# taekkii/deblurgs

Measured on AMD Instinct MI355X. Metric: subframe-renders/sec (fwd+bwd), 1M Gaussians, K=15, 1080p, 1/2/4/8 GPU, higher is better.
Workload: dtype f32; 1 GPU; metric: P=1000000 Gaussians, 1920x1080, K=15 subframes fused, curve_order=3, SH degree 2 (M=9); one blurry view per GPU per step; eager_preferred_steps=279, dropped_steps=0, retried_steps=0, tile_cull=True, depth_output=False, ranks_in_process_group=1

## Files before the change

deblurgs_amd/csrc/api.hip:

```cpp
#include <stdio.h>
#include <string.h>

#include <mutex>
#include <new>

#include "dgs_common.h"

namespace {

thread_local char g_err[512] = "";

int fail(int code, const char* fmt, const char* a = "") {
  snprintf(g_err, sizeof(g_err), fmt, a);
  return code;
}
int fail_hip(hipError_t e, const char* where) {
  snprintf(g_err, sizeof(g_err), "%s: %s", where, hipGetErrorString(e));
  return DGS_E_HIP;
}

constexpr size_t ALIGN = 256;
size_t up(size_t x) { return (x + ALIGN - 1) / ALIGN * ALIGN; }

int sort_bits_for(int W, int H, int K) {
  const uint32_t T = (uint32_t)((W + DGS_TILE - 1) / DGS_TILE) * (uint32_t)((H + DGS_TILE - 1) / DGS_TILE);
  return 32 + (int)dgs_higher_msb(T * (uint32_t)K);
}

DgsLayout make_layout(int P, int W, int H, int K, uint64_t R, bool wide_records, bool forward_only = false) {
  DgsLayout L = {};
  const size_t KP = (size_t)K * (size_t)P;
  const size_t N = (size_t)W * (size_t)H;
  const size_t T = (size_t)((W + DGS_TILE - 1) / DGS_TILE) * (size_t)((H + DGS_TILE - 1) / DGS_TILE);
  size_t o = 0;
  L.geom_rows = o;      o += up(KP * sizeof(DgsRow));
// ... 146 lines not shown
  k->L = make_layout(p->P, p->W, p->H, p->K, R, p->wide_records != 0, p->forward_only != 0);
  if (p->geom_state == nullptr || p->geom_bytes < k->L.geom_total) return fail(DGS_E_CAPACITY, "geom_state too small");
  if ((need & NEED_IMAGE) && (p->image_state == nullptr || p->image_bytes < k->L.image_total))
    return fail(DGS_E_CAPACITY, "image_state too small");
  if ((need & NEED_BINNING) && R > 0 && (p->binning_state == nullptr || p->binning_bytes < k->L.binning_total))
    return fail(DGS_E_CAPACITY, "binning_state too small");
  carve(p, k->L, &k->c);
  k->v = make_view(p, k->L);
  if (io != nullptr) {
    const ScratchLayout sl = scratch_layout(R, p->P, p->K);
    if (io->scratch == nullptr || io->scratch_bytes < sl.total) return fail(DGS_E_CAPACITY, "backward scratch too small");
    char* base = reinterpret_cast<char*>(io->scratch);
    k->contrib = reinterpret_cast<float*>(base);
    k->sums = reinterpret_cast<float*>(base + sl.sums);
    k->partials = reinterpret_cast<double*>(base + sl.partials);
  }
  return DGS_OK;
}

constexpr int PROF_MAX = 16384;
struct Prof {
  bool on = false;
  int n = 0;
  hipEvent_t* beg = nullptr;
  hipEvent_t* end = nullptr;
  int* stage = nullptr;
  int created = 0;
};
}

struct DgsContext {
  std::mutex mu;
  DgsContextOptions opt;
  bool side_ready = false;
  int side_device = -1;
  hipStream_t s2 = nullptr;
  hipEvent_t done[DGS_MAX_BWD_PARTS] = {}, join = nullptr;
  Prof prof;
};

namespace {

int prof_begin(DgsContext* ctx, int stage, hipStream_t s) {
  if (ctx == nullptr || !ctx->prof.on) return -1;
  Prof& pr = ctx->prof;
  std::lock_guard<std::mutex> lk(ctx->mu);
  if (pr.n >= PROF_MAX) return -1;
  const int i = pr.n++;
  if (i >= pr.created) {
    (void)hipEventCreate(&pr.beg[i]);
    (void)hipEventCreate(&pr.end[i]);
    pr.created = i + 1;
  }
  pr.stage[i] = stage;
  (void)hipEventRecord(pr.beg[i], s);
  return i;
}
void prof_end(DgsContext* ctx, int i, hipStream_t s) {
  if (i >= 0) (void)hipEventRecord(ctx->prof.end[i], s);
}

struct StageTimer {
  DgsContext* ctx;
  int id;
  hipStream_t s;
  StageTimer(DgsContext* c, int stage, hipStream_t st) : ctx(c), id(prof_begin(c, stage, st)), s(st) {}
  ~StageTimer() { prof_end(ctx, id, s); }
};

#define DGS_STAGE(stage_id, where, expr)                                   \
// ... 184 lines not shown
  int rc = forward_geometry_impl(p, out, stream, host_dev == nullptr);
  if (rc != DGS_OK) return rc;
  if (p->P > 0) {
    const DgsCarve& c = k.c;
    hipError_t e = dgs_launch_finalize_count(c, p->tile_cull != 0, capacity, out->drop_counter, out->status_dev, host_dev,
                                             out->status_host_indirect, s);
    if (host_dev == nullptr) {
      if (e == hipSuccess && out->drop_counter != nullptr)
        e = hipMemcpyAsync(out->num_rendered_host + 4, out->drop_counter, sizeof(uint32_t), hipMemcpyDeviceToHost, s);
      if (e == hipSuccess)
        e = hipMemcpyAsync(out->num_rendered_host + 2, c.num_rendered + 5, sizeof(uint32_t), hipMemcpyDeviceToHost, s);
      if (e == hipSuccess)
        e = hipMemcpyAsync(out->num_rendered_host + 3, c.num_rendered + 4, sizeof(uint32_t), hipMemcpyDeviceToHost, s);
    }
    if (e != hipSuccess) return fail_hip(e, "finalize count");
  } else {
    out->num_rendered_host[2] = 0;
    out->num_rendered_host[3] = 0;
  }
  return forward_render_impl(p, out, capacity, true, s, phases);
}
int dgs_forward(const DgsProblem* p, const DgsForwardOut* out, uint32_t capacity, dgs_stream_t stream) {
  return forward_capacity_impl(p, out, capacity, stream, 3);
}
int dgs_forward_lists(const DgsProblem* p, const DgsForwardOut* out, uint32_t capacity, dgs_stream_t stream) {
  return forward_capacity_impl(p, out, capacity, stream, 1);
}
int dgs_forward_composite(const DgsProblem* p, const DgsForwardOut* out, uint32_t capacity, dgs_stream_t stream) {
  return forward_render_impl(p, out, capacity, true, reinterpret_cast<hipStream_t>(stream), 2);
}

constexpr int BWD_MAX_PARTS = DGS_MAX_BWD_PARTS;
constexpr uint64_t BWD_OVERLAP_MIN_PAIRS = 4000000;

static hipError_t side_stream(DgsContext* ctx) {
  int dev = 0;
  hipError_t e = hipGetDevice(&dev);
  if (e != hipSuccess) return e;
  if (ctx->side_ready) return dev == ctx->side_device ? hipSuccess : hipErrorInvalidDevice;
  e = hipStreamCreateWithFlags(&ctx->s2, hipStreamNonBlocking);
  for (int i = 0; i < BWD_MAX_PARTS && e == hipSuccess; i++) e = hipEventCreateWithFlags(&ctx->done[i], hipEventDisableTiming);
  if (e == hipSuccess) e = hipEventCreateWithFlags(&ctx->join, hipEventDisableTiming);
  if (e != hipSuccess) {
    for (int i = 0; i < BWD_MAX_PARTS; i++) {
      if (ctx->done[i] != nullptr) (void)hipEventDestroy(ctx->done[i]);
      ctx->done[i] = nullptr;
    }
    if (ctx->join != nullptr) (void)hipEventDestroy(ctx->join);
    if (ctx->s2 != nullptr) (void)hipStreamDestroy(ctx->s2);
    ctx->join = nullptr;
    ctx->s2 = nullptr;
    return e;
  }
  ctx->side_device = dev;
  ctx->side_ready = true;
  return hipSuccess;
}

static int bwd_parts(const DgsContextOptions& opt, int K, int* cut, bool force) {
  int n = 0;
  cut[0] = 0;
  if (opt.bwd_n_parts > 0) {
    for (int i = 0; i < opt.bwd_n_parts && i < BWD_MAX_PARTS - 1 && n < BWD_MAX_PARTS - 1; i++) {
      const int len = opt.bwd_parts[i];
      if (len <= 0 || cut[n] + len >= K) break;
      cut[n + 1] = cut[n] + len;
      n++;
    }
  } else if (K >= 6) {
    cut[1] = (2 * K + 1) / 3;
    cut[2] = K - 1;
    n = 2;
  } else if (force && K >= 2) {
    cut[1] = (K + 1) / 2;
    n = 1;
  }
  cut[++n] = K;
  return n;
}

static hipError_t backward_composite_overlapped(const DgsProblem* p, const DgsBackwardIO* io, const Call& k, hipStream_t s,
                                                const int* cut, int n) {
  const DgsCarve& c = k.c;
  const DgsView& v = k.v;
  DgsContext* ctx = p->context;
  hipStream_t s2 = ctx->s2;
  hipError_t e = hipSuccess;
  bool forked = false;
  for (int i = 0; i < n && e == hipSuccess; i++) {
    e = dgs_launch_composite_bwd(v, c, p->bg, io->dL_dout_color, io->dL_dout_depth, k.contrib, s, cut[i], cut[i + 1]);
    if (i + 1 < n) {
      if (e == hipSuccess) e = hipEventRecord(ctx->done[i], s);
      if (e == hipSuccess) e = hipStreamWaitEvent(s2, ctx->done[i], 0);
      if (e == hipSuccess) {
        forked = true;
        e = dgs_launch_geometry_bwd(*p, v, c, *io, k.contrib, k.sums, k.partials, s2, 1, 0, 0, cut[i], cut[i + 1]);
      }
    }
  }
  if (forked) {
    hipError_t j = hipEventRecord(ctx->join, s2);
    if (j == hipSuccess) j = hipStreamWaitEvent(s, ctx->join, 0);
    if (j != hipSuccess && e == hipSuccess) e = j;
    if (j != hipSuccess) (void)hipStreamSynchronize(s2);
  }
  if (e == hipSuccess) e = dgs_launch_geometry_bwd(*p, v, c, *io, k.contrib, k.sums, k.partials, s, 1, 0, 0, cut[n - 1], cut[n]);
  return e;
}

static int backward_prepare(const DgsProblem* p, const DgsBackwardIO* io, bool all_grads, bool zero_pose, int32_t g_begin,
                            int32_t g_end, hipStream_t s, Call* k, bool* empty) {
  *empty = false;
  int rc = check_problem(p, p != nullptr && p->raw_params != 0);
  if (rc != DGS_OK) return rc;
  if (p->forward_only)
    return fail(DGS_E_ARG, "%s: the problem is forward_only (nothing was kept for a backward)",
                all_grads ? "backward" : "backward_pose_only");
  if (io == nullptr) return fail(DGS_E_ARG, "null DgsBackwardIO");
  if (io->dL_dviewmatrix == nullptr || io->dL_dprojmatrix == nullptr)
    return fail(DGS_E_ARG, "dL_dviewmatrix / dL_dprojmatrix are null");
  if (p->P == 0) {
    *empty = true;
    if (!zero_pose) return DGS_OK;
    hipError_t e = hipMemsetAsync(io->dL_dviewmatrix, 0, (size_t)p->K * 64, s);
    if (e == hipSuccess) e = hipMemsetAsync(io->dL_dprojmatrix, 0, (size_t)p->K * 64, s);
    return e == hipSuccess ? DGS_OK : fail_hip(e, "memset grads");
  }
  if (!all_grads) {
    if (io->dL_dout_color == nullptr || io->radii == nullptr)
      return fail(DGS_E_ARG, "DgsBackwardIO: dL_dout_color / radii are null");
  } else {
    if (io->dL_dout_color == nullptr || io->radii == nullptr || io->dL_dmeans3D == nullptr ||
        (io->dL_dmeans2D == nullptr && io->stats_max_radii2D == nullptr) || io->dL_dcolors == nullptr ||
        io->dL_dopacity == nullptr || io->dL_dcov3D == nullptr)
      return fail(DGS_E_ARG, "DgsBackwardIO: a required pointer is null");
    if (p->shs != nullptr && io->dL_dsh == nullptr) return fail(DGS_E_ARG, "dL_dsh is null");
    if (p->raw_params && p->M > 1 && io->dL_dsh_rest == nullptr) return fail(DGS_E_ARG, "dL_dsh_rest is null");
    if (p->scales != nullptr && (io->dL_dscales == nullptr || io->dL_drotations == nullptr))
      return fail(DGS_E_ARG, "dL_dscales / dL_drotations are null");
    if (g_begin < 0 || g_end > p->P || g_begin > g_end || (g_begin % 256) != 0)
      return fail(DGS_E_ARG, "backward: bad Gaussian range (g_begin must be a multiple of 256)");
  }
  return prepare(p, io->num_rendered, NEED_IMAGE | NEED_BINNING, io, k);
}

static int backward_impl(const DgsProblem* p, const DgsBackwardIO* io, int which, int32_t g_begin, int32_t g_end,
                         hipStream_t s) {
  Call k;
  bool empty;
  const int rc = backward_prepare(p, io, true, (which & 4) != 0, g_begin, g_end, s, &k, &empty);
  if (rc != DGS_OK || empty) return rc;
  const uint64_t R = io->num_rendered;
  int cut[BWD_MAX_PARTS + 1], parts = 1;
  DgsContext* ctx = p->context;
  const int omode = ctx != nullptr ? ctx->opt.bwd_overlap : 0;
  std::unique_lock<std::mutex> side_lock;
  if ((which & 1) && k.v.tile_cull && !p->debug && omode != 0 && !ctx->prof.on && (R >= BWD_OVERLAP_MIN_PAIRS || omode >= 2)) {
    hipStreamCaptureStatus cs = hipStreamCaptureStatusNone;
    if (omode != 3 && hipStreamIsCapturing(s, &cs) != hipSuccess) cs = hipStreamCaptureStatusActive;
    if (cs == hipStreamCaptureStatusNone) parts = bwd_parts(ctx->opt, p->K, cut, omode >= 2);
    if (parts > 1) {
      side_lock = std::unique_lock<std::mutex>(ctx->mu);
      if (side_stream(ctx) != hipSuccess) {
        (void)hipGetLastError();
        side_lock.unlock();
        parts = 1;
      }
    }
  }
  if (parts > 1) {
    hipError_t e = backward_composite_overlapped(p, io, k, s, cut, parts);
    side_lock.unlock();
    if (e != hipSuccess) return fail_hip(e, "composite backward (parts)");
  } else if (which & 1) {
    DGS_STAGE(DGS_STAGE_COMPOSITE_BWD, "composite backward",
              dgs_launch_composite_bwd(k.v, k.c, p->bg, io->dL_dout_color, io->dL_dout_depth, k.contrib, s));
    DGS_STAGE(DGS_STAGE_CONTRIB_REDUCE, "contribution-row totals",
              dgs_launch_geometry_bwd(*p, k.v, k.c, *io, k.contrib, k.sums, k.partials, s, 1, 0, 0));
  }
  if (which & 6)
    DGS_STAGE(DGS_STAGE_GEOMETRY_BWD, "geometry backward",
              dgs_launch_geometry_bwd(*p, k.v, k.c, *io, k.contrib, k.sums, k.partials, s, which & 6, g_begin, g_end));
  return DGS_OK;
}

int dgs_backward(const DgsProblem* p, const DgsBackwardIO* io, dgs_stream_t stream) {
  return backward_impl(p, io, 7, 0, p != nullptr ? p->P : 0, reinterpret_cast<hipStream_t>(stream));
}
int dgs_backward_composite(const DgsProblem* p, const DgsBackwardIO* io, dgs_stream_t stream) {
  return backward_impl(p, io, 1, 0, 0, reinterpret_cast<hipStream_t>(stream));
}
int dgs_backward_geometry(const DgsProblem* p, const DgsBackwardIO* io, int32_t g_begin, int32_t g_end,
                          dgs_stream_t stream) {
  return backward_impl(p, io, 2, g_begin, g_end, reinterpret_cast<hipStream_t>(stream));
}
int32_t dgs_backward_parts(const DgsContext* ctx, int32_t K, uint64_t num_rendered, int32_t tile_cull) {
  const int omode = ctx != nullptr ? ctx->opt.bwd_overlap : 0;
  if (K < 1 || !tile_cull || omode == 0 || (num_rendered < BWD_OVERLAP_MIN_PAIRS && omode < 2)) return 1;
  int cut[BWD_MAX_PARTS + 1];
  return bwd_parts(ctx->opt, K, cut, omode >= 2);
}
int dgs_backward_pose(const DgsProblem* p, const DgsBackwardIO* io, dgs_stream_t stream) {
  return backward_impl(p, io, 4, 0, 0, reinterpret_cast<hipStream_t>(stream));
}

// ... 84 lines not shown
    return fail(DGS_E_ARG, "copy_words: bad argument (at most 4096 words)");
  if (n_words == 0) return DGS_OK;
  hipStream_t s = reinterpret_cast<hipStream_t>(stream);
  void* d = device_view(dst);
  void* sp = device_view(src);
  hipError_t e;
  if (d != nullptr && sp != nullptr)
    e = dgs_launch_copy_words(reinterpret_cast<uint32_t*>(d), reinterpret_cast<const uint32_t*>(sp), n_words, s);
  else
    e = hipMemcpyAsync(dst, src, (size_t)n_words * 4, hipMemcpyDefault, s);
  return e == hipSuccess ? DGS_OK : fail_hip(e, "copy_words");
}

int dgs_context_create(const DgsContextOptions* options, DgsContext** out) {
  if (out == nullptr) return fail(DGS_E_ARG, "context_create: null output");
  *out = nullptr;
  DgsContextOptions o;
  memset(&o, 0, sizeof(o));
  o.bwd_overlap = 1;
  if (options != nullptr) o = *options;
  if (o.bwd_overlap < 0 || o.bwd_overlap > 3 || o.bwd_n_parts < 0 || o.bwd_n_parts > DGS_MAX_BWD_PARTS - 1)
    return fail(DGS_E_ARG, "context_create: bwd_overlap must be 0..3, bwd_n_parts 0..DGS_MAX_BWD_PARTS-1");
  for (int i = 0; i < o.bwd_n_parts; i++)
    if (o.bwd_parts[i] < 1) return fail(DGS_E_ARG, "context_create: a part must hold at least one subframe");
  DgsContext* c = new (std::nothrow) DgsContext();
  if (c == nullptr) return fail(DGS_E_ARG, "context_create: out of host memory");
  c->opt = o;
  *out = c;
  return DGS_OK;
}
int dgs_context_destroy(DgsContext* ctx) {
  if (ctx == nullptr) return DGS_OK;
  hipError_t e = hipSuccess;
  if (ctx->side_ready) {
    e = hipStreamSynchronize(ctx->s2);
    for (int i = 0; i < BWD_MAX_PARTS; i++) (void)hipEventDestroy(ctx->done[i]);
    (void)hipEventDestroy(ctx->join);
    (void)hipStreamDestroy(ctx->s2);
  }
  for (int i = 0; i < ctx->prof.created; i++) {
    (void)hipEventDestroy(ctx->prof.beg[i]);
    (void)hipEventDestroy(ctx->prof.end[i]);
  }
  delete[] ctx->prof.beg;
  delete[] ctx->prof.end;
  delete[] ctx->prof.stage;
  delete ctx;
  return e == hipSuccess ? DGS_OK : fail_hip(e, "context_destroy");
}

int dgs_profile_enable(DgsContext* ctx, int32_t on) {
  if (ctx == nullptr) return fail(DGS_E_ARG, "profile_enable: null context");
  std::lock_guard<std::mutex> lk(ctx->mu);
  if (on) {
    if (ctx->prof.beg == nullptr) ctx->prof.beg = new (std::nothrow) hipEvent_t[PROF_MAX];
    if (ctx->prof.end == nullptr) ctx->prof.end = new (std::nothrow) hipEvent_t[PROF_MAX];
    if (ctx->prof.stage == nullptr) ctx->prof.stage = new (std::nothrow) int[PROF_MAX];
    if (ctx->prof.beg == nullptr || ctx->prof.end == nullptr || ctx->prof.stage == nullptr)
      return fail(DGS_E_ARG, "profile_enable: out of host memory");
  }
  ctx->prof.on = on != 0;
  return DGS_OK;
}
int dgs_profile_reset(DgsContext* ctx) {
  if (ctx == nullptr) return fail(DGS_E_ARG, "profile_reset: null context");
  std::lock_guard<std::mutex> lk(ctx->mu);
  ctx->prof.n = 0;
  return DGS_OK;
}
int dgs_profile_read(DgsContext* ctx, float* ms, int32_t* calls, int32_t n) {
  if (ctx == nullptr) return fail(DGS_E_ARG, "profile_read: null context");
  std::lock_guard<std::mutex> lk(ctx->mu);
// ... 27 lines not shown
```

deblurgs_amd/csrc/composite.hip:

```cpp
#include <type_traits>

#include "dgs_common.h"

namespace {

typedef float v2f __attribute__((ext_vector_type(2)));

constexpr int CW = 4;

struct TileCtx {
  int k, tx, ty;
  uint32_t r0, r1;
};

__device__ __forceinline__ uint32_t xcd_remap(uint32_t b, uint32_t per_xcd) { return (b & 7u) * per_xcd + (b >> 3); }

__device__ __forceinline__ bool load_tile_ctx(const DgsView& v, const uint2* __restrict__ ranges, uint32_t per_xcd,
                                              TileCtx& t) {
  const uint32_t logical = xcd_remap(blockIdx.x, per_xcd);
  const uint32_t gw = logical * CW + (uint32_t)__builtin_amdgcn_readfirstlane((int)(threadIdx.x >> 6));
  const uint32_t KT = (uint32_t)v.K * (uint32_t)v.T;
  if (gw >= KT) return false;
  t.k = (int)(gw / (uint32_t)v.T);
  const uint32_t tile = gw - (uint32_t)t.k * (uint32_t)v.T;
  t.ty = (int)(tile / (uint32_t)v.gx);
  t.tx = (int)(tile - (uint32_t)t.ty * (uint32_t)v.gx);
  const uint2 r = ranges[gw];
  t.r0 = r.x;
  t.r1 = r.y;
  return true;
}

#ifndef DGS_LOG2_CONIC
#define DGS_LOG2_CONIC 0
#endif
#if DGS_LOG2_CONIC
constexpr float K_LOG2E = -1.4426950408889634f;
constexpr float K_HALF_LOG2E = -0.7213475204444817f;
#else
constexpr float K_LOG2E = -1.0f;
constexpr float K_HALF_LOG2E = -0.5f;
#endif
__device__ __forceinline__ float dgs_power2(float A, float B, float C, float dx, float dy) {
  const float u = fmaf(B, dy, A * dx);
#if DGS_LOG2_CONIC
  return fmaf(C * dy, dy, dx * u);
#else
  return fmaf(C * dy, dy, dx * u) * 1.4426950408889634f;
#endif
}

#ifndef DGS_EXACT_POWER
// ... 6 lines not shown
__device__ __forceinline__ float dgs_power_ref(float a, float b, float c, float dx, float dy) {
  const float t0 = __fmul_rn(__fmul_rn(a, dx), dx), t1 = __fmul_rn(__fmul_rn(c, dy), dy);
  const float t2 = __fmul_rn(__fmul_rn(b, dx), dy);
  return __fsub_rn(__fmul_rn(-0.5f, __fadd_rn(t0, t1)), t2);
}
#endif

__device__ __forceinline__ float dgs_min_raw(float c, float x) {
  float r;
  asm("v_min_f32 %0, %1, %2" : "=v"(r) : "v"(c), "v"(x));
  return r;
}

#ifndef DGS_TIMELINE
#define DGS_TIMELINE 0
#endif
#if DGS_TIMELINE
__device__ unsigned long long* g_timeline = nullptr;
#endif

using CullGauss = DgsCull;
#define make_cull dgs_make_cull
#define cull_hit dgs_cull_hit

template <bool WITHDEPTH, bool KEEP, bool CHK = false>
__global__ void __launch_bounds__(64 * CW)
composite_fwd_kernel(DgsView v, uint32_t per_xcd, const uint2* __restrict__ ranges,
                     const uint32_t* __restrict__ point_list, const uint64_t* __restrict__ keys,
                     const DgsRow* __restrict__ rows,
                     const float* __restrict__ bg, float* __restrict__ final_T, uint32_t* __restrict__ n_contrib,
                     float* __restrict__ out_color, float* __restrict__ out_depth, uint32_t* __restrict__ checksum = nullptr) {
  __shared__ float4 s_row[CW][64 * 3];
  TileCtx t;
  if (!load_tile_ctx(v, ranges, per_xcd, t)) return;
  const int lane = dgs_lane(), w = __builtin_amdgcn_readfirstlane((int)(threadIdx.x >> 6));
  const int lx = lane & 7, ly = lane >> 3;
  const int px0 = t.tx * DGS_TILE + lx, py0 = t.ty * DGS_TILE + ly;
  const float pxf0 = (float)px0, pxf1 = (float)(px0 + 8), pyf0 = (float)py0, pyf1 = (float)(py0 + 8);
  const float qx0 = (float)(t.tx * DGS_TILE), qy0 = (float)(t.ty * DGS_TILE);

  float T[4], C0[4], C1[4], C2[4], Dd[4];
  uint32_t last[4], chk[4];
#pragma unroll
  for (int q = 0; q < 4; q++) {
    C0[q] = C1[q] = C2[q] = Dd[q] = 0.0f;
    last[q] = 0;
    chk[q] = 0;
    const int px = px0 + (q & 1) * 8, py = py0 + (q >> 1) * 8;
    T[q] = (px < v.W && py < v.H) ? 1.0f : -1.0f;
  }
  const DgsRow* krows = rows + (size_t)t.k * v.P;
  const uint32_t n = t.r1 - t.r0;
  uint64_t alive[4];
#pragma unroll
  for (int q = 0; q < 4; q++) alive[q] = __ballot(T[q] > 0.0f);

  for (uint32_t base = 0; base < n; base += 64) {
    if ((alive[0] | alive[1] | alive[2] | alive[3]) == 0) break;
    const bool has = base + lane < n;
    float4 A = make_float4(0, 0, 0, 0), B = A, Cc = A;
    if (has) {
      const uint32_t g = v.pack_tile_shift > 0
                             ? (uint32_t)(keys[t.r0 + base + lane] >> v.pack_g_shift) &
                                   ((1u << (v.pack_tile_shift - v.pack_g_shift)) - 1u)
                             : point_list[t.r0 + base + lane];
      const float4* rp = reinterpret_cast<const float4*>(krows + g);
      A = rp[0];
// ... 65 lines not shown
    }
    };
    if ((~pdm & mu_all) == 0ull)
      run_batch(std::false_type{});
    else
      run_batch(std::true_type{});
#pragma unroll
    for (int q = 0; q < 4; q++) alive[q] = __ballot(T[q] > 0.0f);
    __builtin_amdgcn_wave_barrier();
  }

  const float bg0 = bg[0], bg1 = bg[1], bg2 = bg[2];
  const size_t N = (size_t)v.W * v.H;
#pragma unroll
  for (int q = 0; q < 4; q++) {
    const int px = px0 + (q & 1) * 8, py = py0 + (q >> 1) * 8;
    if (px < v.W && py < v.H) {
      const size_t pix = (size_t)py * v.W + px;
      const float Tf = fabsf(T[q]);
      if (KEEP) {
        final_T[(size_t)t.k * N + pix] = Tf;
        n_contrib[(size_t)t.k * N + pix] = last[q];
      }
      float* oc = out_color + (size_t)t.k * 3 * N;
      oc[pix] = C0[q] + Tf * bg0;
      oc[N + pix] = C1[q] + Tf * bg1;
      oc[2 * N + pix] = C2[q] + Tf * bg2;
      if (WITHDEPTH) out_depth[(size_t)t.k * N + pix] = Dd[q] + Tf * v.z_far;
      if (CHK) checksum[(size_t)t.k * N + pix] = chk[q];
    }
  }
}

template <bool TIGHT, bool HASDEPTH, bool POSE = false>
__global__ void __launch_bounds__(64 * CW)
composite_bwd_kernel(DgsView v, uint32_t per_xcd, const uint2* __restrict__ ranges,
                     const uint32_t* __restrict__ point_list, const uint64_t* __restrict__ keys,
                     const DgsRow* __restrict__ rows,
                     const float* __restrict__ bg, const float* __restrict__ final_T,
                     const uint32_t* __restrict__ n_contrib, const float* __restrict__ dL_dpix,
                     const float* __restrict__ dL_ddepth, const uint32_t* __restrict__ dup_off,
                     float* __restrict__ contrib) {
  __shared__ float4 s_row[CW][64 * 3];
  __shared__ __attribute__((aligned(16))) float s_part[CW][10][68];
  TileCtx t;
  if (!load_tile_ctx(v, ranges, per_xcd, t)) return;
#if DGS_TIMELINE
  const unsigned long long t_begin = wall_clock64();
#endif
  const int lane = dgs_lane(), w = __builtin_amdgcn_readfirstlane((int)(threadIdx.x >> 6));
  const int lx = lane & 7, ly = lane >> 3;
  const int px0 = t.tx * DGS_TILE + lx, py0 = t.ty * DGS_TILE + ly;
  const float pxf0 = (float)px0, pxf1 = (float)(px0 + 8), pyf0 = (float)py0, pyf1 = (float)(py0 + 8);
  const float qx0 = (float)(t.tx * DGS_TILE), qy0 = (float)(t.ty * DGS_TILE);
  const size_t N = (size_t)v.W * v.H;
  const float bg0 = bg[0], bg1 = bg[1], bg2 = bg[2];
  const int rrow = lane >> 2, rq = lane & 3;
  const bool rlane = rrow < (POSE ? (HASDEPTH ? 6 : 5) : (HASDEPTH ? 10 : 9));
  float* const contrib_lane = contrib + (rrow < 10 ? rrow : 0);
  static_assert(sizeof(float) * 68 == 272, "the store offsets below are multiples of one s_part row");
  const uint32_t part_base = (uint32_t)__builtin_amdgcn_readfirstlane((int)(uint32_t)(size_t)(&s_part[w][0][0]));
  

  float T[4];
  v2f gA[4], gB[4];
  float accg[4];
  uint32_t last[4];
  uint32_t maxc = 0;
#pragma unroll
  for (int q = 0; q < 4; q++) {
    const int px = px0 + (q & 1) * 8, py = py0 + (q >> 1) * 8;
    const bool inside = (px < v.W && py < v.H);
    const size_t pix = (size_t)py * v.W + px;
    const float Tfin = inside ? final_T[(size_t)t.k * N + pix] : 0.0f;
    T[q] = Tfin;
    last[q] = inside ? n_contrib[(size_t)t.k * N + pix] : 0u;
    const float* gp = dL_dpix + (size_t)t.k * 3 * N;
    const float g0 = inside ? gp[pix] : 0.0f;
    const float g1 = inside ? gp[N + pix] : 0.0f;
// ... 237 lines not shown
}
#endif

static uint32_t per_xcd_blocks(const DgsView& v) {
  const uint64_t KT = (uint64_t)v.K * v.T;
  const uint64_t nblk = (KT + CW - 1) / CW;
  return (uint32_t)((nblk + 7) / 8);
}

hipError_t dgs_launch_composite_fwd(const DgsView& v, const DgsCarve& c, const float* bg, float* out_color,
                                    float* out_depth, hipStream_t s, uint32_t* checksum) {
  const uint32_t per = per_xcd_blocks(v);
  if (per == 0) return hipSuccess;
#define DGS_CFWD(WD, KP)                                                                                                  \
  hipLaunchKernelGGL((composite_fwd_kernel<WD, KP>), dim3(per * 8), dim3(64 * CW), 0, s, v, per, c.ranges, c.point_list, \
                     c.keys_sorted, c.rows, bg, c.final_T, c.n_contrib, out_color, out_depth)
  const bool keep = c.final_T != nullptr && c.n_contrib != nullptr;
  if (checksum != nullptr) {
    if (out_depth == nullptr || !keep) return hipErrorInvalidValue;
    hipLaunchKernelGGL((composite_fwd_kernel<true, true, true>), dim3(per * 8), dim3(64 * CW), 0, s, v, per, c.ranges,
                       c.point_list, c.keys_sorted, c.rows, bg, c.final_T, c.n_contrib, out_color, out_depth, checksum);
    return hipGetLastError();
  }
  if (out_depth != nullptr) {
    if (keep) DGS_CFWD(true, true); else DGS_CFWD(true, false);
  } else {
    if (keep) DGS_CFWD(false, true); else DGS_CFWD(false, false);
  }
#undef DGS_CFWD
  return hipGetLastError();
}

hipError_t dgs_launch_composite_bwd(const DgsView& v_all, const DgsCarve& c, const float* bg, const float* dL_dpix,
                                    const float* dL_ddepth, float* contrib, hipStream_t s, int k0, int k1, bool pose) {
  if (k1 < 0) { k0 = 0; k1 = v_all.K; }
  DgsView v = v_all;
  v.K = k1 - k0;
  const size_t N = (size_t)v.W * v.H;
  const uint32_t per = per_xcd_blocks(v);
  if (per == 0) return hipSuccess;
  const uint2* ranges = c.ranges + (size_t)k0 * v.T;
  const DgsRow* rows = c.rows + (size_t)k0 * v.P;
  const float* final_T = c.final_T + (size_t)k0 * N;
  const uint32_t* n_contrib = c.n_contrib + (size_t)k0 * N;
  dL_dpix += (size_t)k0 * 3 * N;
  if (dL_ddepth != nullptr) dL_ddepth += (size_t)k0 * N;
#define DGS_CBWD(TI, HD, ...)                                                                                       \
  hipLaunchKernelGGL((composite_bwd_kernel<TI, HD, ##__VA_ARGS__>), dim3(per * 8), dim3(64 * CW), 0, s, v, per, ranges, c.point_list, \
                     c.keys_sorted, rows, bg, final_T, n_contrib, dL_dpix, dL_ddepth, c.point_offsets, contrib)
  if (pose) {
    if (v.tile_cull) {
      if (dL_ddepth != nullptr) DGS_CBWD(true, true, true); else DGS_CBWD(true, false, true);
    } else {
      if (dL_ddepth != nullptr) DGS_CBWD(false, true, true); else DGS_CBWD(false, false, true);
    }
  } else if (v.tile_cull) {
    if (dL_ddepth != nullptr) DGS_CBWD(true, true); else DGS_CBWD(true, false);
  } else {
    if (dL_ddepth != nullptr) DGS_CBWD(false, true); else DGS_CBWD(false, false);
  }
#undef DGS_CBWD
  return hipGetLastError();
}
```

deblurgs_amd/csrc/dgs_common.h:

```cpp
#pragma once
#include <hip/hip_runtime.h>
#include <stdint.h>

#include "../../include/dgs_hip.h"

#define DGS_TILE 16
#define DGS_DEPTH_KEY_BASE 0x3E4CCCCDu
#define DGS_ROW_F 12
#define DGS_CONTRIB_F 12
#define DGS_SUMS_F 16
#define DGS_WAVE 64

struct __attribute__((aligned(16))) DgsRow {
  float x, y;
  float cx, cy, cz, op;
  float r, g, b, depth;
  uint32_t dup_offset;
  int32_t radius;
};
static_assert(sizeof(DgsRow) == 4 * DGS_ROW_F, "row must be 48 bytes");

struct DgsCarve {
  DgsRow* rows;
  float* cov3D;
// ... 49 lines not shown
  maxx = min(gx, max(0, (int)((px + max_radius + DGS_TILE - 1) / DGS_TILE)));
  maxy = min(gy, max(0, (int)((py + max_radius + DGS_TILE - 1) / DGS_TILE)));
}

template <int CTRL, int ROW_MASK>
__device__ __forceinline__ float dgs_dpp(float v) {
  return __int_as_float(__builtin_amdgcn_update_dpp(0, __float_as_int(v), CTRL, ROW_MASK, 0xf, false));
}

__device__ __forceinline__ float dgs_wave_sum63(float v) {
  v += dgs_dpp<0xB1, 0xf>(v);
  v += dgs_dpp<0x4E, 0xf>(v);
  v += dgs_dpp<0x141, 0xf>(v);
  v += dgs_dpp<0x140, 0xf>(v);
  v += dgs_dpp<0x142, 0xa>(v);
  v += dgs_dpp<0x143, 0xc>(v);
  return v;
}

__device__ __forceinline__ int dgs_lane() { return (int)(threadIdx.x & 63); }

__device__ __forceinline__ float dgs_quad_sum(float v) {
  v += dgs_dpp<0xB1, 0xf>(v);
  v += dgs_dpp<0x4E, 0xf>(v);
  return v;
}
__device__ __forceinline__ float dgs_row_sum(float v) {
  v += dgs_dpp<0xB1, 0xf>(v);
  v += dgs_dpp<0x4E, 0xf>(v);
  v += dgs_dpp<0x141, 0xf>(v);
  v += dgs_dpp<0x140, 0xf>(v);
  return v;
}

__device__ __forceinline__ float dgs_sgn(float x) { return (x > 0.0f) ? 1.0f : ((x < 0.0f) ? -1.0f : 0.0f); }

constexpr double DGS_TOTALS_FX = 16777216.0;
template <typename T>
__device__ __forceinline__ bool dgs_totals_publish(T a, T c, float* __restrict__ work, unsigned long long& t0,
                                                   unsigned long long& t1, bool& bad) {
  unsigned long long* acc = reinterpret_cast<unsigned long long*>(work + 2);
  unsigned int* flag = reinterpret_cast<unsigned int*>(work + 7);
  const bool fin = __builtin_isfinite(a) && __builtin_isfinite(c) && a < (T)5.0e11 && c < (T)5.0e11;
  if (!fin) {
    atomicOr(flag, 1u);
  } else {
    const unsigned long long ia = (unsigned long long)__double2ll_rn((double)a * DGS_TOTALS_FX);
    const unsigned long long ic = (unsigned long long)__double2ll_rn((double)c * DGS_TOTALS_FX);
    const unsigned long long oa = atomicAdd(&acc[0], ia), oc = atomicAdd(&acc[1], ic);
    if (oa + ia < oa || oc + ic < oc) atomicOr(flag, 1u);
  }
  __threadfence();
  const unsigned int ticket = atomicAdd(reinterpret_cast<unsigned int*>(work + 6), 1u);
  if (ticket != gridDim.x - 1) return false;
  __threadfence();
  t0 = atomicAdd(&acc[0], 0ull);
  t1 = atomicAdd(&acc[1], 0ull);
  bad = atomicOr(flag, 0u) != 0u;
  return true;
}

int dgs_fail_arg(const char* msg);
int dgs_fail_hip(hipError_t e, const char* where);

struct DgsView {
  int P, D, M, W, H, K;
// ... 50 lines not shown
  float qm = fminf(x_out ? qx : big, y_out ? qy : big);
  qm = (x_out || y_out) ? qm : 0.0f;
  return !(qm * 0.9999f > g.r2);
}

hipError_t dgs_launch_preprocess(const DgsProblem& p, const DgsView& v, const DgsCarve& c, int32_t* radii,
                                 hipStream_t s);
hipError_t dgs_launch_mark_visible(int P, const float* means3D, const float* view, uint8_t* present, hipStream_t s);
hipError_t dgs_launch_cloud_activations(int P, const float* scales, const float* rotations, const float* opacities,
                                        float scale_lb, float* out_scales, float* out_rotations, float* out_opacities,
                                        hipStream_t s);
hipError_t dgs_launch_finalize_count(const DgsCarve& c, int cull, uint32_t cap, uint32_t* drops, uint32_t* status,
                                     uint32_t* host_words, const uint64_t* host_indirect, hipStream_t s);
hipError_t dgs_launch_clear_words(uint32_t* p, int n, hipStream_t s);
hipError_t dgs_launch_copy_words(uint32_t* dst, const uint32_t* src, int n, hipStream_t s);
hipError_t dgs_launch_ranges(const DgsView& v, const DgsCarve& c, uint32_t R, hipStream_t s,
                             const uint32_t* n_dev = nullptr, int tile_shift = 32);
hipError_t dgs_launch_scan(const uint32_t* in, uint32_t* out, uint64_t n, uint32_t* tmp, uint32_t* total,
                           hipStream_t s);
hipError_t dgs_launch_sort(uint64_t* keys, uint32_t* vals, uint64_t* keys_alt, uint32_t* vals_alt, uint64_t n,
                           int begin_bit, int end_bit, uint32_t* tmp, int* result_in_alt, hipStream_t s,
                           const uint32_t* n_dev = nullptr);
hipError_t dgs_launch_duplicate_sorted(const DgsView& v, const DgsCarve& c, const uint32_t* order, uint32_t* tt_sorted,
                                       uint32_t* offs_sorted, uint32_t* scan_tmp, uint32_t cap, hipStream_t s);
hipError_t dgs_launch_cull_count(const DgsView& v, const DgsCarve& c, hipStream_t s);
hipError_t dgs_launch_cull_offsets(const DgsView& v, const DgsCarve& c, uint32_t* total_tight, hipStream_t s,
                                   bool counts_in_order = false);
hipError_t dgs_launch_duplicate_tight(const DgsView& v, const DgsCarve& c, const uint32_t* order, uint32_t cap,
                                      hipStream_t s);
hipError_t dgs_launch_composite_fwd(const DgsView& v, const DgsCarve& c, const float* bg, float* out_color,
                                    float* out_depth, hipStream_t s, uint32_t* checksum = nullptr);
hipError_t dgs_launch_composite_bwd(const DgsView& v, const DgsCarve& c, const float* bg, const float* dL_dpix,
                                    const float* dL_ddepth, float* contrib, hipStream_t s, int k0 = 0, int k1 = -1,
                                    bool pose = false);
hipError_t dgs_launch_geometry_bwd(const DgsProblem& p, const DgsView& v, const DgsCarve& c, const DgsBackwardIO& io,
                                   const float* contrib, float* sums, double* partials, hipStream_t s, int phases,
                                   int g_begin, int g_end, int k0 = 0, int k1 = -1);
hipError_t dgs_launch_geometry_pose_bwd(const DgsProblem& p, const DgsView& v, const DgsCarve& c, const DgsBackwardIO& io,
                                        const float* contrib, float* sums, double* partials, hipStream_t s, int phases);
hipError_t dgs_launch_depth_sort(uint32_t* keys, uint32_t* keys_alt, uint32_t* order, uint32_t* order_alt, int K,
                                 uint32_t P, uint32_t* tmp, uint32_t* vis_dst, uint32_t* wide_flag, hipStream_t s,
                                 const uint32_t* cnt_src = nullptr, uint32_t* cnt_dst = nullptr,
                                 bool drop_invisible = false);
size_t dgs_depth_sort_tmp_words(int K, uint32_t P);
size_t dgs_scan_tmp_words(uint64_t n);
size_t dgs_sort_tmp_words(uint64_t n);
int dgs_sort_num_passes(int begin_bit, int end_bit);
int dgs_geometry_bwd_blocks(int P);
```

deblurgs_amd/csrc/geometry_bwd.hip:

```cpp
#include "dgs_common.h"


namespace {

__device__ const float SH_C0 = 0.28209479177387814f;
__device__ const float SH_C1 = 0.4886025119029199f;
__device__ const float SH_C2[] = {1.0925484305920792f, -1.0925484305920792f, 0.31539156525252005f,
                                  -1.0925484305920792f, 0.5462742152960396f};
__device__ const float SH_C3[] = {-0.5900435899266435f, 2.890611442640554f, -0.4570457994644658f,
                                  0.3731763325901154f, -0.4570457994644658f, 1.445305721320277f,
                                  -0.5900435899266435f};

constexpr int GB_THREADS = 256;
constexpr int NMAT = 24;

struct M3 {
  float m[3][3];
};
__device__ __forceinline__ M3 mul(const M3& A, const M3& B) {
  M3 R;
#pragma unroll
  for (int c = 0; c < 3; c++)
#pragma unroll
    for (int r = 0; r < 3; r++) R.m[c][r] = A.m[0][r] * B.m[c][0] + A.m[1][r] * B.m[c][1] + A.m[2][r] * B.m[c][2];
  return R;
}
__device__ __forceinline__ M3 tr(const M3& A) {
  M3 R;
#pragma unroll
  for (int c = 0; c < 3; c++)
#pragma unroll
    for (int r = 0; r < 3; r++) R.m[c][r] = A.m[r][c];
  return R;
}
__device__ __forceinline__ float sigmoidf_(float x) { return 1.0f / (1.0f + expf(-x)); }

template <int NPARTS = 3>
__global__ void __launch_bounds__(256)
contrib_reduce_kernel(uint64_t n, const uint32_t* __restrict__ status, const uint32_t* __restrict__ order,
                      const uint32_t* __restrict__ tt_visible, const uint32_t* __restrict__ tiles,
                      const uint32_t* __restrict__ offsets, const float* __restrict__ contrib,
                      float* __restrict__ sums) {
  if (status[5] != 0u) return;
  const uint64_t t = (uint64_t)blockIdx.x * 256 + threadIdx.x;
  const uint64_t j = t >> 2;
  const uint32_t part = (uint32_t)t & 3u;
  if (j >= n || (part == 3u && DGS_SUMS_F < 16)) return;
  if (NPARTS < 3 && part >= (uint32_t)NPARTS) return;
  const uint32_t vis = tt_visible[j], nt = tiles[j], off = offsets[j], dst = order[j];
  if (vis == 0u) return;
  float4 a = make_float4(0.0f, 0.0f, 0.0f, 0.0f);
  if (nt > 0 && part < (uint32_t)NPARTS) {
    const float4* cp = reinterpret_cast<const float4*>(contrib + (size_t)off * DGS_CONTRIB_F) + part;
    float4 q0 = cp[0], q1 = a, q2 = a, q3 = a;
    if (nt > 1) q1 = cp[3];
    if (nt > 2) q2 = cp[6];
    if (nt > 3) q3 = cp[9];
    a = q0;
    if (nt > 1) { a.x += q1.x; a.y += q1.y; a.z += q1.z; a.w += q1.w; }
    if (nt > 2) { a.x += q2.x; a.y += q2.y; a.z += q2.z; a.w += q2.w; }
    if (nt > 3) { a.x += q3.x; a.y += q3.y; a.z += q3.z; a.w += q3.w; }
    uint32_t r = 4;
    for (; r + 8 <= nt; r += 8) {
      float4 q[8];
#pragma unroll
      for (int i = 0; i < 8; i++) q[i] = cp[3 * (r + i)];
#pragma unroll
      for (int i = 0; i < 8; i++) {
        a.x += q[i].x;
        a.y += q[i].y;
        a.z += q[i].z;
        a.w += q[i].w;
      }
    }
    for (; r < nt; r++) {
      const float4 q = cp[3 * r];
      a.x += q.x;
      a.y += q.y;
      a.z += q.z;
      a.w += q.w;
    }
  }
  reinterpret_cast<float4*>(sums + (size_t)dst * DGS_SUMS_F)[part] = a;
}

#define DGS_SH_BACKWARD(PS)  \
  {  \
        const float* cam = campos + 3 * k;  \
        const float dox = mx - cam[0], doy = my - cam[1], doz = mz - cam[2];  \
        const float len = sqrtf(dox * dox + doy * doy + doz * doz);  \
        const float x = dox / len, y = doy / len, z = doz / len;  \
        float dRGB[3];  \
_Pragma("unroll")  \
        for (int ch = 0; ch < 3; ch++) {  \
          const float psv = (PS)[ch];  \
          float f = psv;  \
          if (v.use_sigmoid) {  \
            const float sg = sigmoidf_(psv);  \
            f = sg * (1.0f - sg);  \
          }  \
          dRGB[ch] = dcol[ch] * f;  \
        }  \
        float ddir[3] = {0, 0, 0};    \
        float cf[MAXC];    \
        cf[0] = SH_C0;  \
        if (MAXC > 1 && ncoef > 1) {  \
          cf[1] = -SH_C1 * y;  \
          cf[2] = SH_C1 * z;  \
          cf[3] = -SH_C1 * x;  \
_Pragma("unroll")  \
          for (int ch = 0; ch < 3; ch++) {  \
            ddir[0] += (-SH_C1 * sh[9 + ch]) * dRGB[ch];  \
            ddir[1] += (-SH_C1 * sh[3 + ch]) * dRGB[ch];  \
            ddir[2] += (SH_C1 * sh[6 + ch]) * dRGB[ch];  \
          }  \
        }  \
// ... 790 lines not shown
```

Baseline: 1426 subframe-renders/sec.

## Fold per-part contrib reduction into composite backward launches as ride-along blocks

Drops the side stream and events that ran the contribution reduction for each finished subframe part alongside the composite backward. Instead, each later composite backward launch gets extra leading blocks, sized by CU count, that grid-stride over the previous part's reduction inside the same kernel. Only the last part's reduction runs as a separate launch. This removes event and stream-wait overhead and the capture check, and lets the overlap work under graph capture. The cost is a larger, shared kernel with a different occupancy hint, and reduction blocks competing with tile blocks for CUs.

```diff
diff --git a/deblurgs_amd/csrc/api.hip b/deblurgs_amd/csrc/api.hip
--- a/deblurgs_amd/csrc/api.hip
+++ b/deblurgs_amd/csrc/api.hip
@@ -1,6 +1,7 @@
 #include <stdio.h>
 #include <string.h>
 
+#include <atomic>
 #include <mutex>
 #include <new>
 
@@ -213,10 +214,7 @@
 struct DgsContext {
   std::mutex mu;
   DgsContextOptions opt;
-  bool side_ready = false;
-  int side_device = -1;
-  hipStream_t s2 = nullptr;
-  hipEvent_t done[DGS_MAX_BWD_PARTS] = {}, join = nullptr;
+  std::atomic<uint32_t> ride_blocks{0};
   Prof prof;
 };
 
@@ -467,28 +465,22 @@
 
 constexpr int BWD_MAX_PARTS = DGS_MAX_BWD_PARTS;
 constexpr uint64_t BWD_OVERLAP_MIN_PAIRS = 4000000;
-
-static hipError_t side_stream(DgsContext* ctx) {
-  int dev = 0;
-  hipError_t e = hipGetDevice(&dev);
-  if (e != hipSuccess) return e;
-  if (ctx->side_ready) return dev == ctx->side_device ? hipSuccess : hipErrorInvalidDevice;
-  e = hipStreamCreateWithFlags(&ctx->s2, hipStreamNonBlocking);
-  for (int i = 0; i < BWD_MAX_PARTS && e == hipSuccess; i++) e = hipEventCreateWithFlags(&ctx->done[i], hipEventDisableTiming);
-  if (e == hipSuccess) e = hipEventCreateWithFlags(&ctx->join, hipEventDisableTiming);
-  if (e != hipSuccess) {
-    for (int i = 0; i < BWD_MAX_PARTS; i++) {
-      if (ctx->done[i] != nullptr) (void)hipEventDestroy(ctx->done[i]);
-      ctx->done[i] = nullptr;
-    }
-    if (ctx->join != nullptr) (void)hipEventDestroy(ctx->join);
-    if (ctx->s2 != nullptr) (void)hipStreamDestroy(ctx->s2);
-    ctx->join = nullptr;
-    ctx->s2 = nullptr;
-    return e;
-  }
-  ctx->side_device = dev;
-  ctx->side_ready = true;
+#ifndef DGS_RIDE_BLOCKS_PER_CU
+#define DGS_RIDE_BLOCKS_PER_CU 2
+#endif
+
+static hipError_t ride_blocks(DgsContext* ctx, uint32_t* nred) {
+  uint32_t n = ctx->ride_blocks.load(std::memory_order_relaxed);
+  if (n == 0) {
+    int dev = 0, cus = 0;
+    hipError_t e = hipGetDevice(&dev);
+    if (e == hipSuccess) e = hipDeviceGetAttribute(&cus, hipDeviceAttributeMultiprocessorCount, dev);
+    if (e != hipSuccess) return e;
+    if (cus < 1) return hipErrorInvalidDevice;
+    n = ((uint32_t)cus * DGS_RIDE_BLOCKS_PER_CU + 7u) & ~7u;
+    ctx->ride_blocks.store(n, std::memory_order_relaxed);
+  }
+  *nred = n;
   return hipSuccess;
 }
 
@@ -515,29 +507,14 @@
 }
 
 static hipError_t backward_composite_overlapped(const DgsProblem* p, const DgsBackwardIO* io, const Call& k, hipStream_t s,
-                                                const int* cut, int n) {
+                                                const int* cut, int n, uint32_t nred) {
   const DgsCarve& c = k.c;
   const DgsView& v = k.v;
-  DgsContext* ctx = p->context;
-  hipStream_t s2 = ctx->s2;
   hipError_t e = hipSuccess;
-  bool forked = false;
   for (int i = 0; i < n && e == hipSuccess; i++) {
-    e = dgs_launch_composite_bwd(v, c, p->bg, io->dL_dout_color, io->dL_dout_depth, k.contrib, s, cut[i], cut[i + 1]);
-    if (i + 1 < n) {
-      if (e == hipSuccess) e = hipEventRecord(ctx->done[i], s);
-      if (e == hipSuccess) e = hipStreamWaitEvent(s2, ctx->done[i], 0);
-      if (e == hipSuccess) {
-        forked = true;
-        e = dgs_launch_geometry_bwd(*p, v, c, *io, k.contrib, k.sums, k.partials, s2, 1, 0, 0, cut[i], cut[i + 1]);
-      }
-    }
-  }
-  if (forked) {
-    hipError_t j = hipEventRecord(ctx->join, s2);
-    if (j == hipSuccess) j = hipStreamWaitEvent(s, ctx->join, 0);
-    if (j != hipSuccess && e == hipSuccess) e = j;
-    if (j != hipSuccess) (void)hipStreamSynchronize(s2);
+    const DgsRide ride = {nred, i > 0 ? cut[i - 1] : 0, i > 0 ? cut[i] : 0, k.sums};
+    e = dgs_launch_composite_bwd(v, c, p->bg, io->dL_dout_color, io->dL_dout_depth, k.contrib, s, cut[i], cut[i + 1], false,
+                                 i > 0 ? &ride : nullptr);
   }
   if (e == hipSuccess) e = dgs_launch_geometry_bwd(*p, v, c, *io, k.contrib, k.sums, k.partials, s, 1, 0, 0, cut[n - 1], cut[n]);
   return e;
@@ -587,25 +564,18 @@
   if (rc != DGS_OK || empty) return rc;
   const uint64_t R = io->num_rendered;
   int cut[BWD_MAX_PARTS + 1], parts = 1;
+  uint32_t nred = 0;
   DgsContext* ctx = p->context;
   const int omode = ctx != nullptr ? ctx->opt.bwd_overlap : 0;
-  std::unique_lock<std::mutex> side_lock;
   if ((which & 1) && k.v.tile_cull && !p->debug && omode != 0 && !ctx->prof.on && (R >= BWD_OVERLAP_MIN_PAIRS || omode >= 2)) {
-    hipStreamCaptureStatus cs = hipStreamCaptureStatusNone;
-    if (omode != 3 && hipStreamIsCapturing(s, &cs) != hipSuccess) cs = hipStreamCaptureStatusActive;
-    if (cs == hipStreamCaptureStatusNone) parts = bwd_parts(ctx->opt, p->K, cut, omode >= 2);
-    if (parts > 1) {
-      side_lock = std::unique_lock<std::mutex>(ctx->mu);
-      if (side_stream(ctx) != hipSuccess) {
-        (void)hipGetLastError();
-        side_lock.unlock();
-        parts = 1;
-      }
+    parts = bwd_parts(ctx->opt, p->K, cut, omode >= 2);
+    if (parts > 1 && ride_blocks(ctx, &nred) != hipSuccess) {
+      (void)hipGetLastError();
+      parts = 1;
     }
   }
   if (parts > 1) {
-    hipError_t e = backward_composite_overlapped(p, io, k, s, cut, parts);
-    side_lock.unlock();
+    hipError_t e = backward_composite_overlapped(p, io, k, s, cut, parts, nred);
     if (e != hipSuccess) return fail_hip(e, "composite backward (parts)");
   } else if (which & 1) {
     DGS_STAGE(DGS_STAGE_COMPOSITE_BWD, "composite backward",
@@ -756,12 +726,6 @@
 int dgs_context_destroy(DgsContext* ctx) {
   if (ctx == nullptr) return DGS_OK;
   hipError_t e = hipSuccess;
-  if (ctx->side_ready) {
-    e = hipStreamSynchronize(ctx->s2);
-    for (int i = 0; i < BWD_MAX_PARTS; i++) (void)hipEventDestroy(ctx->done[i]);
-    (void)hipEventDestroy(ctx->join);
-    (void)hipStreamDestroy(ctx->s2);
-  }
   for (int i = 0; i < ctx->prof.created; i++) {
     (void)hipEventDestroy(ctx->prof.beg[i]);
     (void)hipEventDestroy(ctx->prof.end[i]);
diff --git a/deblurgs_amd/csrc/composite.hip b/deblurgs_amd/csrc/composite.hip
--- a/deblurgs_amd/csrc/composite.hip
+++ b/deblurgs_amd/csrc/composite.hip
@@ -16,8 +16,8 @@
 __device__ __forceinline__ uint32_t xcd_remap(uint32_t b, uint32_t per_xcd) { return (b & 7u) * per_xcd + (b >> 3); }
 
 __device__ __forceinline__ bool load_tile_ctx(const DgsView& v, const uint2* __restrict__ ranges, uint32_t per_xcd,
-                                              TileCtx& t) {
-  const uint32_t logical = xcd_remap(blockIdx.x, per_xcd);
+                                              TileCtx& t, uint32_t block) {
+  const uint32_t logical = xcd_remap(block, per_xcd);
   const uint32_t gw = logical * CW + (uint32_t)__builtin_amdgcn_readfirstlane((int)(threadIdx.x >> 6));
   const uint32_t KT = (uint32_t)v.K * (uint32_t)v.T;
   if (gw >= KT) return false;
@@ -90,7 +90,7 @@
                      float* __restrict__ out_color, float* __restrict__ out_depth, uint32_t* __restrict__ checksum = nullptr) {
   __shared__ float4 s_row[CW][64 * 3];
   TileCtx t;
-  if (!load_tile_ctx(v, ranges, per_xcd, t)) return;
+  if (!load_tile_ctx(v, ranges, per_xcd, t, blockIdx.x)) return;
   const int lane = dgs_lane(), w = __builtin_amdgcn_readfirstlane((int)(threadIdx.x >> 6));
   const int lx = lane & 7, ly = lane >> 3;
   const int px0 = t.tx * DGS_TILE + lx, py0 = t.ty * DGS_TILE + ly;
@@ -222,19 +222,26 @@
   }
 }
 
-template <bool TIGHT, bool HASDEPTH, bool POSE = false>
-__global__ void __launch_bounds__(64 * CW)
+template <bool TIGHT, bool HASDEPTH, bool POSE = false, bool RIDE = false>
+__global__ void __launch_bounds__(64 * CW) __attribute__((amdgpu_waves_per_eu(RIDE && !HASDEPTH ? 6 : 1)))
 composite_bwd_kernel(DgsView v, uint32_t per_xcd, const uint2* __restrict__ ranges,
                      const uint32_t* __restrict__ point_list, const uint64_t* __restrict__ keys,
                      const DgsRow* __restrict__ rows,
                      const float* __restrict__ bg, const float* __restrict__ final_T,
                      const uint32_t* __restrict__ n_contrib, const float* __restrict__ dL_dpix,
                      const float* __restrict__ dL_ddepth, const uint32_t* __restrict__ dup_off,
-                     float* __restrict__ contrib) {
+                     float* __restrict__ contrib, DgsRideArgs ride) {
   __shared__ float4 s_row[CW][64 * 3];
   __shared__ __attribute__((aligned(16))) float s_part[CW][10][68];
+  if (RIDE && blockIdx.x < ride.nred) {
+    if (ride.status[5] != 0u) return;
+    dgs_contrib_reduce_range<3>(ride.j0, ride.nj, (uint64_t)blockIdx.x * (64 * CW) + threadIdx.x,
+                                (uint64_t)ride.nred * (64 * CW), ride.order, ride.tt_visible, ride.tiles, ride.offsets,
+                                contrib, ride.sums);
+    return;
+  }
   TileCtx t;
-  if (!load_tile_ctx(v, ranges, per_xcd, t)) return;
+  if (!load_tile_ctx(v, ranges, per_xcd, t, RIDE ? blockIdx.x - ride.nred : blockIdx.x)) return;
 #if DGS_TIMELINE
   const unsigned long long t_begin = wall_clock64();
 #endif
@@ -538,7 +545,8 @@
 }
 
 hipError_t dgs_launch_composite_bwd(const DgsView& v_all, const DgsCarve& c, const float* bg, const float* dL_dpix,
-                                    const float* dL_ddepth, float* contrib, hipStream_t s, int k0, int k1, bool pose) {
+                                    const float* dL_ddepth, float* contrib, hipStream_t s, int k0, int k1, bool pose,
+                                    const DgsRide* ride) {
   if (k1 < 0) { k0 = 0; k1 = v_all.K; }
   DgsView v = v_all;
   v.K = k1 - k0;
@@ -551,10 +559,25 @@
   const uint32_t* n_contrib = c.n_contrib + (size_t)k0 * N;
   dL_dpix += (size_t)k0 * 3 * N;
   if (dL_ddepth != nullptr) dL_ddepth += (size_t)k0 * N;
+  DgsRideArgs ra = {};
+  if (ride != nullptr && ride->nred > 0 && ride->k1 > ride->k0) {
+    if (pose || !v.tile_cull || (ride->nred & 7u) != 0u) return hipErrorInvalidValue;
+    ra.nred = ride->nred;
+    ra.j0 = (uint64_t)ride->k0 * v.P;
+    ra.nj = (uint64_t)(ride->k1 - ride->k0) * v.P;
+    ra.status = c.num_rendered;
+    ra.order = c.gsort_vals;
+    ra.tt_visible = c.tt_sorted;
+    ra.tiles = c.tt_tight;
+    ra.offsets = c.offs_tight;
+    ra.sums = ride->sums;
+  }
 #define DGS_CBWD(TI, HD, ...)                                                                                       \
-  hipLaunchKernelGGL((composite_bwd_kernel<TI, HD, ##__VA_ARGS__>), dim3(per * 8), dim3(64 * CW), 0, s, v, per, ranges, c.point_list, \
-                     c.keys_sorted, rows, bg, final_T, n_contrib, dL_dpix, dL_ddepth, c.point_offsets, contrib)
-  if (pose) {
+  hipLaunchKernelGGL((composite_bwd_kernel<TI, HD, ##__VA_ARGS__>), dim3(per * 8 + ra.nred), dim3(64 * CW), 0, s, v, per, ranges, \
+                     c.point_list, c.keys_sorted, rows, bg, final_T, n_contrib, dL_dpix, dL_ddepth, c.point_offsets, contrib, ra)
+  if (ra.nred > 0) {
+    if (dL_ddepth != nullptr) DGS_CBWD(true, true, false, true); else DGS_CBWD(true, false, false, true);
+  } else if (pose) {
     if (v.tile_cull) {
       if (dL_ddepth != nullptr) DGS_CBWD(true, true, true); else DGS_CBWD(true, false, true);
     } else {
diff --git a/deblurgs_amd/csrc/dgs_common.h b/deblurgs_amd/csrc/dgs_common.h
--- a/deblurgs_amd/csrc/dgs_common.h
+++ b/deblurgs_amd/csrc/dgs_common.h
@@ -105,6 +105,72 @@
   v += dgs_dpp<0x140, 0xf>(v);
   return v;
 }
+
+template <int NPARTS>
+__device__ __forceinline__ void dgs_contrib_reduce_range(uint64_t j0, uint64_t nj, uint64_t t0, uint64_t stride,
+                                                         const uint32_t* __restrict__ order,
+                                                         const uint32_t* __restrict__ tt_visible,
+                                                         const uint32_t* __restrict__ tiles,
+                                                         const uint32_t* __restrict__ offsets,
+                                                         const float* __restrict__ contrib, float* __restrict__ sums) {
+  for (uint64_t t = t0; t < 4 * nj; t += stride) {
+    const uint64_t j = j0 + (t >> 2);
+    const uint32_t part = (uint32_t)t & 3u;
+    if (part == 3u && DGS_SUMS_F < 16) continue;
+    if (NPARTS < 3 && part >= (uint32_t)NPARTS) continue;
+    const uint32_t vis = tt_visible[j], nt = tiles[j], off = offsets[j], dst = order[j];
+    if (vis == 0u) continue;
+    float4 a = make_float4(0.0f, 0.0f, 0.0f, 0.0f);
+    if (nt > 0 && part < (uint32_t)NPARTS) {
+      const float4* cp = reinterpret_cast<const float4*>(contrib + (size_t)off * DGS_CONTRIB_F) + part;
+      float4 q0 = cp[0], q1 = a, q2 = a, q3 = a;
+      if (nt > 1) q1 = cp[3];
+      if (nt > 2) q2 = cp[6];
+      if (nt > 3) q3 = cp[9];
+      a = q0;
+      if (nt > 1) { a.x += q1.x; a.y += q1.y; a.z += q1.z; a.w += q1.w; }
+      if (nt > 2) { a.x += q2.x; a.y += q2.y; a.z += q2.z; a.w += q2.w; }
+      if (nt > 3) { a.x += q3.x; a.y += q3.y; a.z += q3.z; a.w += q3.w; }
+      uint32_t r = 4;
+      for (; r + 8 <= nt; r += 8) {
+        float4 q[8];
+#pragma unroll
+        for (int i = 0; i < 8; i++) q[i] = cp[3 * (r + i)];
+#pragma unroll
+        for (int i = 0; i < 8; i++) {
+          a.x += q[i].x;
+          a.y += q[i].y;
+          a.z += q[i].z;
+          a.w += q[i].w;
+        }
+      }
+      for (; r < nt; r++) {
+        const float4 q = cp[3 * r];
+        a.x += q.x;
+        a.y += q.y;
+        a.z += q.z;
+        a.w += q.w;
+      }
+    }
+    reinterpret_cast<float4*>(sums + (size_t)dst * DGS_SUMS_F)[part] = a;
+  }
+}
+
+struct DgsRideArgs {
+  uint32_t nred;
+  uint64_t j0, nj;
+  const uint32_t* status;
+  const uint32_t* order;
+  const uint32_t* tt_visible;
+  const uint32_t* tiles;
+  const uint32_t* offsets;
+  float* sums;
+};
+struct DgsRide {
+  uint32_t nred;
+  int k0, k1;
+  float* sums;
+};
 
 __device__ __forceinline__ float dgs_sgn(float x) { return (x > 0.0f) ? 1.0f : ((x < 0.0f) ? -1.0f : 0.0f); }
 
@@ -221,7 +287,7 @@
                                     float* out_depth, hipStream_t s, uint32_t* checksum = nullptr);
 hipError_t dgs_launch_composite_bwd(const DgsView& v, const DgsCarve& c, const float* bg, const float* dL_dpix,
                                     const float* dL_ddepth, float* contrib, hipStream_t s, int k0 = 0, int k1 = -1,
-                                    bool pose = false);
+                                    bool pose = false, const DgsRide* ride = nullptr);
 hipError_t dgs_launch_geometry_bwd(const DgsProblem& p, const DgsView& v, const DgsCarve& c, const DgsBackwardIO& io,
                                    const float* contrib, float* sums, double* partials, hipStream_t s, int phases,
                                    int g_begin, int g_end, int k0 = 0, int k1 = -1);
diff --git a/deblurgs_amd/csrc/geometry_bwd.hip b/deblurgs_amd/csrc/geometry_bwd.hip
--- a/deblurgs_amd/csrc/geometry_bwd.hip
+++ b/deblurgs_amd/csrc/geometry_bwd.hip
@@ -42,46 +42,8 @@
                       const uint32_t* __restrict__ offsets, const float* __restrict__ contrib,
                       float* __restrict__ sums) {
   if (status[5] != 0u) return;
-  const uint64_t t = (uint64_t)blockIdx.x * 256 + threadIdx.x;
-  const uint64_t j = t >> 2;
-  const uint32_t part = (uint32_t)t & 3u;
-  if (j >= n || (part == 3u && DGS_SUMS_F < 16)) return;
-  if (NPARTS < 3 && part >= (uint32_t)NPARTS) return;
-  const uint32_t vis = tt_visible[j], nt = tiles[j], off = offsets[j], dst = order[j];
-  if (vis == 0u) return;
-  float4 a = make_float4(0.0f, 0.0f, 0.0f, 0.0f);
-  if (nt > 0 && part < (uint32_t)NPARTS) {
-    const float4* cp = reinterpret_cast<const float4*>(contrib + (size_t)off * DGS_CONTRIB_F) + part;
-    float4 q0 = cp[0], q1 = a, q2 = a, q3 = a;
-    if (nt > 1) q1 = cp[3];
-    if (nt > 2) q2 = cp[6];
-    if (nt > 3) q3 = cp[9];
-    a = q0;
-    if (nt > 1) { a.x += q1.x; a.y += q1.y; a.z += q1.z; a.w += q1.w; }
-    if (nt > 2) { a.x += q2.x; a.y += q2.y; a.z += q2.z; a.w += q2.w; }
-    if (nt > 3) { a.x += q3.x; a.y += q3.y; a.z += q3.z; a.w += q3.w; }
-    uint32_t r = 4;
-    for (; r + 8 <= nt; r += 8) {
-      float4 q[8];
-#pragma unroll
-      for (int i = 0; i < 8; i++) q[i] = cp[3 * (r + i)];
-#pragma unroll
-      for (int i = 0; i < 8; i++) {
-        a.x += q[i].x;
-        a.y += q[i].y;
-        a.z += q[i].z;
-        a.w += q[i].w;
-      }
-    }
-    for (; r < nt; r++) {
-      const float4 q = cp[3 * r];
-      a.x += q.x;
-      a.y += q.y;
-      a.z += q.z;
-      a.w += q.w;
-    }
-  }
-  reinterpret_cast<float4*>(sums + (size_t)dst * DGS_SUMS_F)[part] = a;
+  dgs_contrib_reduce_range<NPARTS>(0, n, (uint64_t)blockIdx.x * 256 + threadIdx.x, (uint64_t)gridDim.x * 256, order,
+                                   tt_visible, tiles, offsets, contrib, sums);
 }
 
 #define DGS_SH_BACKWARD(PS)  \
```

Result: no change. 1435 subframe-renders/sec, median of 6 (+0.6%).
